# duanyiqun/DiffusionDepth

Measured on NVIDIA H100. Metric: depth maps/sec @ KITTI 352x1216, Swin-L, 20 DDIM steps, higher is better.
Workload: dtype f32 (fp32-grade products on wgmma: 3-pass fp16 split, fp32 accumulate)

## Files before the change

### diffusiondepth_b200/csrc/engine.cu

```cuda
#include <cuda.h>
#include <cuda_runtime.h>
#include <math.h>
#include <stdio.h>
#include <stdlib.h>
#include <string.h>

#include <algorithm>
#include <map>
#include <string>
#include <vector>

#include "../../include/dd_engine.h"
#include "kernels.cuh"
#include "convgen.cuh"
#include "conv_halo.cuh"
#include "pred_fold.cuh"
#include "swin.cuh"
#include "mpvit.cuh"
#include "backward.cuh"
#include "codec_train.cuh"
#include "producer_train.cuh"

namespace {

// ... 289 lines not shown
  float* UP[3] = {nullptr, nullptr, nullptr};
  bool resample = false;
  float* UPR[3] = {nullptr, nullptr, nullptr};
  float* KS = nullptr;
};
struct ResBlockW {
  GenLayer c1, c2, ds;
  bool has_ds = false;
};
struct ResNetW {
  bool enabled = false, ready = false;
  int H = 0, W = 0;
  int depths[4] = {0, 0, 0, 0}, C[4] = {64, 128, 256, 512}, Hs[4] = {0, 0, 0, 0}, Ws[4] = {0, 0, 0, 0};
  std::vector<ResBlockW> blocks[4];
  Planes IN, T, Yp[2];
  float* Y32[2] = {nullptr, nullptr};
  float* D32 = nullptr;
};

struct DwLayer {
  int C = 0, K = 3;
  float* w = nullptr;
  float* bias = nullptr;
  int bn = -1;
  float *raw_w = nullptr, *raw_bias = nullptr;
};
struct MpBlockW {
  float *ln1_g = nullptr, *ln1_b = nullptr, *ln2_g = nullptr, *ln2_b = nullptr;
  GenLayer qkv, proj, fc1, fc2;
};
struct MpEncoderW {
  DwLayer cpe;
  float* crpe_w = nullptr;
  float* crpe_b = nullptr;
  std::vector<MpBlockW> layers;
};
struct MpStageW {
  DwLayer pe_dw[4], inv_dw;
  GenLayer pe_pw[4], inv1, inv2, agg;
  MpEncoderW enc[4];
};
constexpr int kMpHeads = 8;
constexpr int kMpChunksMax = 256;
struct FactorAttBufs {
  float *part_m = nullptr, *part_s = nullptr, *colinv = nullptr, *part_ktv = nullptr, *ktv = nullptr;
};
struct MPViTW {
  bool enabled = false, ready = false;
  int H = 0, W = 0, heads = kMpHeads, mlp_ratio = 4;
  int dims[4] = {0, 0, 0, 0}, out_dims[4] = {0, 0, 0, 0}, layers[4] = {0, 0, 0, 0}, paths[4] = {0, 0, 0, 0};
  int Hs[4] = {0, 0, 0, 0}, Ws[4] = {0, 0, 0, 0};
  GenLayer stem0, stem1;
  MpStageW stage[4];
  Planes IN, S1, D, EP0, AP, HP, CAT;
  float* XS = nullptr;
  float* E[4] = {nullptr, nullptr, nullptr, nullptr};
  float* R1 = nullptr;
  float* QKV = nullptr;
  FactorAttBufs fab;
};

struct DropPathState {
  int mask[4] = {0, 0, 0, 0}, blocks = 0;
  bool on = false;
  float* scales = nullptr;
};

}

struct dd_engine {
  dd_config cfg;
  int sm_count = 0;
  bool weights_ready = false;
  bool packed = false;
  std::map<std::string, Raw> raw;
  ConvLayer L[12];
  struct Fold {
    __half* w = nullptr;
    float* bias = nullptr;
    float wscale = 1.f;
    float* src[2] = {nullptr, nullptr};
    double* k5 = nullptr;
    float* k5_abs = nullptr;
  } fold;
  float* w_flip[6] = {};
  float* amax = nullptr;
  PackStage* stage = nullptr;
  cudaEvent_t pack_done = nullptr;
  float* gn_gamma[4] = {nullptr, nullptr, nullptr, nullptr};
  float* gn_beta[4] = {nullptr, nullptr, nullptr, nullptr};
  float* temb = nullptr;
  float* dec_wt = nullptr;
  float* dec_bt = nullptr;
  float* dec_wc = nullptr;
  float dec_bc = 0.f;
  float* dec_wu = nullptr;
  float* dec_bu = nullptr;
  float* dec_bn = nullptr;
  float *enc_w1 = nullptr, *enc_b1 = nullptr, *enc_w2 = nullptr, *enc_b2 = nullptr;
  int codec_mode = DD_CODEC_EVAL;
  struct CodecTrain {
    float *dec_gb = nullptr;
    float *dec_wt = nullptr, *dec_bt = nullptr, *dec_bn = nullptr;
    float* zero16 = nullptr;
    float *enc_w1 = nullptr, *enc_w2 = nullptr, *enc_gb = nullptr;
    float *enc_w1f = nullptr, *enc_b1f = nullptr, *enc_w2f = nullptr, *enc_b2f = nullptr;
    double *part = nullptr, *sum1 = nullptr;
    double *sums = nullptr, *part_db = nullptr;
    float* rec = nullptr;
    int nrec = 0;
  } ct;
  int producer_mode = DD_PRODUCER_EVAL;
  struct ProdBn {
    GenLayer raw;
    float *gamma = nullptr, *beta = nullptr;
    int C = 0;
    int stage = 0;
    long long n = 0;
    bool fresh = false;
    size_t rec_off = 0;
    std::string key;
  };
  struct ProdTrain {
    std::vector<ProdBn> layers;
    float* U = nullptr;
    double *part = nullptr, *sum1 = nullptr;
    float *s = nullptr, *t = nullptr, *rec = nullptr;
    size_t rec_floats = 0;
  } pt;
  struct BnSync {
    dd_allgather_fn fn = nullptr;
    void* user = nullptr;
    int world = 1;
    int cap = 0;
    double *row = nullptr, *rows = nullptr, *tot1 = nullptr, *tot2 = nullptr;
  } sync;
  std::vector<void*> owned;
  std::vector<int64_t> ts;
  std::vector<float> cx, ce;
  void* ws = nullptr;
  float *x32 = nullptr, *Y = nullptr, *cond = nullptr, *mr[4] = {}, *temb_sel = nullptr;
  double* stats[4] = {};
  __half *xs_hi = nullptr, *xs_lo = nullptr, *S_hi[2] = {}, *S_lo[2] = {};
  int* status = nullptr;
  struct Bwd {
    float *y1 = nullptr, *y2 = nullptr, *y5 = nullptr, *y6 = nullptr;
    Planes a1, f0, fa, fp, a5;
    float *g[2] = {nullptr, nullptr};
    Planes gp;
    float *gn_part = nullptr, *ab = nullptr, *col_part = nullptr, *dtemb = nullptr, *dcond = nullptr;
    float *scales = nullptr, *amax = nullptr;
    double* wg_part = nullptr;
  } bw;
  struct LoopBwd {
    float* stash = nullptr;
    float* gl = nullptr;
    float* stage = nullptr;
    double* acc = nullptr;
    double* acc_cond = nullptr;
    float *z = nullptr, *r = nullptr, *du = nullptr;
    double *part_act = nullptr, *part_wc = nullptr, *part_wt = nullptr;
  } lp;
  int stats_tiles_img[4] = {0, 0, 0, 0};
  Producers prod;
  Backbone bb;
  ResNetW rn;
// ... 398 lines not shown
  return launched(e, "gn_finalize");
}

template <int C, int COND>
void launch_apply(const dd::ApplyArgs& a, int B, int up_qpb, cudaStream_t st) {
  if (COND == 2 && C == 256) {
    if (up_qpb == 4) {
      dim3 grid((a.W / 2 + 1 + 3) / 4, a.H / 2 + 1, B);
      dd::gn_apply_up_split_kernel<4, 4><<<grid, 256, 0, st>>>(a);
    } else {
      dim3 grid(a.W / 2 + 1, a.H / 2 + 1, B);
      dd::gn_apply_up_split_kernel<4, 1><<<grid, 64, 0, st>>>(a);
    }
  } else {
    constexpr int PPB = 256 / (C / 8);
    dim3 grid((a.H * a.W + PPB - 1) / PPB, B);
    dd::gn_apply_split_kernel<C, COND><<<grid, 256, 0, st>>>(a);
  }
}

template <int C, int COND>
int run_apply(dd_engine* e, int which, const float* temb, int temb_bstride, __half* out_hi, __half* out_lo,
              cudaStream_t st, const float* y = nullptr) {
  const Geom g = geom_of(e->cfg);
  dd::ApplyArgs a;
  a.y = y != nullptr ? y : e->Y;
  a.mean_rstd = e->mr[which];
  a.gamma = e->gn_gamma[which];
  a.beta = e->gn_beta[which];
  a.cond = e->cond;
  a.temb = temb;
  a.temb_bstride = temb_bstride;
  a.H = g.h;
  a.W = g.w;
  a.ch = e->cfg.cond_h;
  a.cw = e->cfg.cond_w;
  a.ry = g.h > 1 ? static_cast<float>(a.ch - 1) / static_cast<float>(g.h - 1) : 0.f;
  a.rx = g.w > 1 ? static_cast<float>(a.cw - 1) / static_cast<float>(g.w - 1) : 0.f;
  a.out_hi = out_hi;
  a.out_lo = out_lo;
  a.scale = kActScale;
  a.status = e->status;
  launch_apply<C, COND>(a, g.B, 4, st);
  return launched(e, "gn_apply");
}

bool fold_active(const dd_engine* e) {
  return e->cfg.variant == DD_VARIANT_SWIN && !(e->cfg.flags & (DD_FLAG_SIMT_CONV | DD_FLAG_CHAIN_PRED));
}
int ring_blocks_per_img(const Geom& g) {
  return std::min(dd::ring_segments(g.h, g.w), g.tiles_max / g.B);
}

int run_fold(dd_engine* e, cudaStream_t st) {
  const Geom g = geom_of(e->cfg);
  int rc;
  CUtensorMap m_hi, m_lo;
  if ((rc = make_patch_map(&m_hi, e->S_hi[0], g.B, g.h, g.w))) return rc;
  if ((rc = make_patch_map(&m_lo, e->S_lo[0], g.B, g.h, g.w))) return rc;
  dd::FoldArgs a;
  a.B = g.B;
  a.H = g.h;
  a.W = g.w;
  a.tiles_x = (g.w + dd::F5_TW - 1) / dd::F5_TW;
  a.tiles_y = (g.h + dd::F5_TH - 1) / dd::F5_TH;
  a.num_tiles = a.tiles_x * a.tiles_y * g.B;
  a.w = e->fold.w;
  a.bias = e->fold.bias;
  a.acc_scale = 1.f / (kActScale * e->fold.wscale);
  a.y32 = e->Y;
  a.stats_partial = e->stats[2];
  e->stats_tiles_img[2] = a.tiles_x * a.tiles_y;
  const int grid = std::min(a.num_tiles, e->sm_count);
  dd::conv5x5_fold_kernel<<<grid, dd::F5::THREADS, dd::F5::SMEM_BYTES, st>>>(m_hi, m_lo, a);
  if ((rc = launched(e, "conv5x5_fold"))) return rc;
  dd::RingArgs r;
  r.H = g.h;
  r.W = g.w;
  r.nseg = dd::ring_segments(g.h, g.w);
  r.blocks_per_img = ring_blocks_per_img(g);
  r.a_hi = e->S_hi[0];
  r.a_lo = e->S_lo[0];
  r.a_inv_scale = 1.f / kActScale;
  r.wb = e->L[3].w_simt;
  r.bb = e->L[3].bias;
  r.wp = e->L[4].w_simt;
  r.y32 = e->Y;
  r.ring_partial = e->stats[3];
  dd::ring_fix_kernel<<<dim3(r.blocks_per_img, g.B), dd::RING_THREADS, dd::RING_SMEM, st>>>(r);
  return launched(e, "ring_fix");
}

int run_tail(dd_engine* e, float cx, float ce, float* eps_out, cudaStream_t st);

void launch_final(const dd::FinalArgs& f, int B, cudaStream_t st) {
  dim3 grid((f.P * 4 + 255) / 256, B);
  dd::gn_relu_ddim_kernel<<<grid, 256, 0, st>>>(f);
}

int run_step(dd_engine* e, const float* temb, int temb_bstride, float cx, float ce, float* eps_out, cudaStream_t st) {
  const Geom g = geom_of(e->cfg);
  int rc;
  if ((rc = run_conv(e, 0, e->xs_hi, e->xs_lo, kXScale, dd::EPI_F32_STATS, e->Y, e->stats[0], nullptr, nullptr, st))) return rc;
  if ((rc = run_finalize(e, 0, 64, st))) return rc;
  if ((rc = run_apply<64, 0>(e, 0, nullptr, 0, e->S_hi[0], e->S_lo[0], st))) return rc;
  if ((rc = run_conv(e, 1, e->S_hi[0], e->S_lo[0], kActScale, dd::EPI_F32_STATS, e->Y, e->stats[1], nullptr, nullptr, st)))
    return rc;
  if ((rc = run_finalize(e, 1, 256, st))) return rc;
  const __half *p_hi, *p_lo;
  if (e->cfg.variant == DD_VARIANT_SWIN) {
    if ((rc = run_apply<256, 2>(e, 1, temb, temb_bstride, e->S_hi[1], e->S_lo[1], st))) return rc;
    if ((rc = run_conv(e, 2, e->S_hi[1], e->S_lo[1], kActScale, dd::EPI_SPLIT, nullptr, nullptr, e->S_hi[0], e->S_lo[0], st)))
      return rc;
    if (fold_active(e)) {
      if ((rc = run_fold(e, st))) return rc;
      if ((rc = run_finalize(e, 2, 64, st, e->stats[3], ring_blocks_per_img(g)))) return rc;
      return run_tail(e, cx, ce, eps_out, st);
    }
    if ((rc = run_conv(e, 3, e->S_hi[0], e->S_lo[0], kActScale, dd::EPI_SPLIT, nullptr, nullptr, e->S_hi[1], e->S_lo[1], st)))
      return rc;
    p_hi = e->S_hi[1];
    p_lo = e->S_lo[1];
  } else {
    if ((rc = run_apply<256, 1>(e, 1, temb, temb_bstride, e->S_hi[1], e->S_lo[1], st))) return rc;
    p_hi = e->S_hi[1];
    p_lo = e->S_lo[1];
  }
  if ((rc = run_conv(e, 4, p_hi, p_lo, kActScale, dd::EPI_F32_STATS, e->Y, e->stats[2], nullptr, nullptr, st))) return rc;
  if ((rc = run_finalize(e, 2, 64, st))) return rc;
  return run_tail(e, cx, ce, eps_out, st);
}

int run_tail(dd_engine* e, float cx, float ce, float* eps_out, cudaStream_t st) {
  const Geom g = geom_of(e->cfg);
  int rc;
  if ((rc = run_apply<64, 0>(e, 2, nullptr, 0, e->S_hi[0], e->S_lo[0], st))) return rc;
  if ((rc = run_conv(e, 5, e->S_hi[0], e->S_lo[0], kActScale, dd::EPI_F32_STATS, e->Y, e->stats[3], nullptr, nullptr, st))) return rc;
  if ((rc = run_finalize(e, 3, 16, st))) return rc;
  dd::FinalArgs f;
  f.y = e->Y;
  f.mean_rstd = e->mr[3];
  f.gamma = e->gn_gamma[3];
  f.beta = e->gn_beta[3];
  f.x = e->x32;
  f.x_hi = e->xs_hi;
  f.x_lo = e->xs_lo;
  f.eps_out = eps_out;
  f.cx = cx;
  f.ce = ce;
  f.scale = kXScale;
  f.P = g.P;
  f.status = e->status;
  launch_final(f, g.B, st);
  return launched(e, "gn_relu_ddim");
}

int transpose_in(const float* nchw, float* nhwc, int B, int C, int P, cudaStream_t st) {
  dim3 grid((P + 31) / 32, (C + 31) / 32, B), block(32, 8);
  dd::nchw_to_nhwc_kernel<<<grid, block, 0, st>>>(nchw, nhwc, C, P);
  return check_launch("nchw_to_nhwc");
}
int transpose_out(const float* nhwc, float* nchw, int B, int C, int P, cudaStream_t st) {
  dim3 grid((P + 31) / 32, (C + 31) / 32, B), block(32, 8);
  dd::nhwc_to_nchw_kernel<<<grid, block, 0, st>>>(nhwc, nchw, C, P);
  return check_launch("nhwc_to_nchw");
}
int split_planes(dd_engine* e, const float* x, __half* hi, __half* lo, size_t n, float scale, cudaStream_t st) {
  dd::split_planes_kernel<<<grid_of(n / 4), 256, 0, st>>>(x, hi, lo, n / 4, scale, e->status);
  return check_launch("split_planes");
// ... 145 lines not shown
int bn_fold(const float* const* bn, int ch, std::vector<float>& scale, std::vector<float>& shift, cudaStream_t st) {
  std::vector<float> v[4];
  for (int i = 0; i < 4; ++i) {
    v[i].resize(ch);
    CUDA_TRY(cudaMemcpyAsync(v[i].data(), bn[i], ch * 4, cudaMemcpyDeviceToHost, st));
  }
  CUDA_TRY(cudaStreamSynchronize(st));
  scale.resize(ch);
  shift.resize(ch);
  const float* host[4] = {v[0].data(), v[1].data(), v[2].data(), v[3].data()};
  bn_fold_host(host, ch, scale.data(), shift.data());
  return DD_OK;
}
int find_bn(dd_engine* e, const std::string& prefix, const float** bn) {
  const char* parts[4] = {".weight", ".bias", ".running_mean", ".running_var"};
  for (int i = 0; i < 4; ++i) {
    const Raw* r = find(e, prefix + parts[i]);
    if (!r) return fail(DD_ERR_INVALID, "missing weights: " + prefix + parts[i]);
    bn[i] = r->ptr;
  }
  return DD_OK;
}
int copy_param(dd_engine* e, const std::string& key, size_t n, float** out, cudaStream_t st) {
  const Raw* r = find(e, key);
  if (!r) return fail(DD_ERR_INVALID, "missing weights: " + key);
  size_t have = 1;
  for (int64_t d : r->shape) have *= static_cast<size_t>(d);
  if (have != n) return fail(DD_ERR_INVALID, "weight shape mismatch: " + key);
  int rc;
  if ((rc = dev_alloc(e, reinterpret_cast<void**>(out), n * 4))) return rc;
  CUDA_TRY(cudaMemcpyAsync(*out, r->ptr, n * 4, cudaMemcpyDeviceToDevice, st));
  return DD_OK;
}

const char* const kGnKey[4] = {"model.noise_embedding.1", "model.noise_embedding.4", "model.pred.1", "model.pred.4"};
constexpr int kGnCh[4] = {64, 256, 64, 16};
const std::string kDecPrefix = "depth_transform.conv_inv_transform.";
const std::string kEncPrefix = "depth_transform.conv_transform.";
struct CodecKey {
  const char* leaf;
  size_t host_off;
  std::vector<int64_t> shape;
};
#define DD_STAGE_OFF(m) (offsetof(PackStage, m) / sizeof(float))
const CodecKey kDecKeys[8] = {{"0.weight", DD_STAGE_OFF(dec_wt), {16, 16, 4, 4}}, {"0.bias", DD_STAGE_OFF(dec_bt), {16}},
                              {"1.weight", DD_STAGE_OFF(dec_g), {16}},            {"1.bias", DD_STAGE_OFF(dec_be), {16}},
                              {"1.running_mean", DD_STAGE_OFF(dec_mu), {16}},     {"1.running_var", DD_STAGE_OFF(dec_var), {16}},
                              {"3.0.weight", DD_STAGE_OFF(dec_wc), {1, 16, 3, 3}}, {"3.0.bias", DD_STAGE_OFF(dec_bc), {1}}};
const CodecKey kEncKeys[10] = {
    {"0.0.weight", DD_STAGE_OFF(enc_w1), {16, 1, 3, 3}},        {"0.1.weight", DD_STAGE_OFF(enc_bn1[0]), {16}},
    {"0.1.bias", DD_STAGE_OFF(enc_bn1[1]), {16}},               {"0.1.running_mean", DD_STAGE_OFF(enc_bn1[2]), {16}},
    {"0.1.running_var", DD_STAGE_OFF(enc_bn1[3]), {16}},        {"1.0.weight", DD_STAGE_OFF(enc_w2), {16, 16, 3, 3}},
    {"1.1.weight", DD_STAGE_OFF(enc_bn2[0]), {16}},             {"1.1.bias", DD_STAGE_OFF(enc_bn2[1]), {16}},
    {"1.1.running_mean", DD_STAGE_OFF(enc_bn2[2]), {16}},       {"1.1.running_var", DD_STAGE_OFF(enc_bn2[3]), {16}}};
#undef DD_STAGE_OFF
size_t numel(const std::vector<int64_t>& s) {
  size_t n = 1;
  for (int64_t d : s) n *= static_cast<size_t>(d);
  return n;
}

int alloc_pack(dd_engine* h, bool encoder, cudaStream_t st) {
  const bool swin = h->cfg.variant == DD_VARIANT_SWIN;
  int rc;
  if ((rc = dev_array(h, &h->amax, 16))) return rc;
  for (int i = 0; i < 6; ++i) {
    if (!swin && (i == 2 || i == 3)) continue;
    const int co = kConvCout[i], ci = kConvCin[i];
    if ((rc = alloc_layer(h, h->L[i], co, ci))) return rc;
    if (has_backward(h->cfg)) {
      if ((rc = dev_array(h, &h->w_flip[i], static_cast<size_t>(co) * ci * 9))) return rc;
      if ((rc = alloc_layer(h, h->L[6 + i], ci, co))) return rc;
      CUDA_TRY(cudaMemsetAsync(h->L[6 + i].bias, 0, ci * 4, st));
    }
  }
  if (fold_active(h)) {
    const size_t n5 = 64 * 256 * 25;
    if ((rc = dev_array(h, &h->fold.w, dd::F5::W_ELEMS))) return rc;
    if ((rc = dev_array(h, &h->fold.bias, 64))) return rc;
    if ((rc = dev_array(h, &h->fold.src[0], 256 * 256 * 9))) return rc;
    if ((rc = dev_array(h, &h->fold.src[1], 64 * 256 * 9))) return rc;
    if ((rc = dev_array(h, &h->fold.k5, n5))) return rc;
    if ((rc = dev_array(h, &h->fold.k5_abs, n5))) return rc;
  }
  for (int i = 0; i < 4; ++i) {
    if ((rc = dev_array(h, &h->gn_gamma[i], kGnCh[i]))) return rc;
    if ((rc = dev_array(h, &h->gn_beta[i], kGnCh[i]))) return rc;
  }
  if ((rc = dev_array(h, &h->temb, DD_TIME_ROWS * 256))) return rc;
  if ((rc = dev_array(h, &h->dec_wt, 4 * 4 * 16 * 16))) return rc;
  if ((rc = dev_array(h, &h->dec_bt, 16))) return rc;
  if ((rc = dev_array(h, &h->dec_wc, 9 * 16))) return rc;
  if ((rc = dev_array(h, &h->dec_wu, 4 * 4 * 16 * 16))) return rc;
  if ((rc = dev_array(h, &h->dec_bu, 16))) return rc;
  if ((rc = dev_array(h, &h->dec_bn, 3 * 16))) return rc;
  dd_engine::CodecTrain& ct = h->ct;
  if ((rc = dev_array(h, &ct.dec_gb, 2 * 16))) return rc;
  if ((rc = dev_array(h, &ct.dec_wt, 4 * 4 * 16 * 16))) return rc;
  if ((rc = dev_array(h, &ct.dec_bt, 16))) return rc;
  if ((rc = dev_array(h, &ct.dec_bn, 3 * 16))) return rc;
  if ((rc = dev_array(h, &ct.zero16, 16))) return rc;
  CUDA_TRY(cudaMemsetAsync(ct.zero16, 0, 16 * 4, st));
  const Geom g = geom_of(h->cfg);
  if ((rc = dev_array(h, &ct.part, static_cast<size_t>(codec_stats_blocks(static_cast<long long>(g.B) * g.P * 4)) *
                                         dd::BNS_COLS)))
    return rc;
  if ((rc = dev_array(h, &ct.sum1, 16))) return rc;
  if ((rc = dev_array(h, &ct.sums, 32))) return rc;
  if ((rc = dev_array(h, &ct.part_db, static_cast<size_t>(dec_act_blocks(g)) * 16))) return rc;
  if ((rc = dev_array(h, &ct.rec, static_cast<size_t>(std::max(h->cfg.num_inference_steps, 2)) * 32))) return rc;
  ct.nrec = 0;
  h->enc_w1 = nullptr;
  if (encoder) {
    if ((rc = dev_array(h, &h->enc_w1, 144))) return rc;
    if ((rc = dev_array(h, &h->enc_b1, 16))) return rc;
    if ((rc = dev_array(h, &h->enc_w2, 2304))) return rc;
    if ((rc = dev_array(h, &h->enc_b2, 16))) return rc;
    if ((rc = dev_array(h, &ct.enc_w1, 144))) return rc;
    if ((rc = dev_array(h, &ct.enc_w2, 2304))) return rc;
    if ((rc = dev_array(h, &ct.enc_gb, 4 * 16))) return rc;
    if ((rc = dev_array(h, &ct.enc_w1f, 144))) return rc;
    if ((rc = dev_array(h, &ct.enc_b1f, 16))) return rc;
    if ((rc = dev_array(h, &ct.enc_w2f, 2304))) return rc;
    if ((rc = dev_array(h, &ct.enc_b2f, 16))) return rc;
  }
  return DD_OK;
}

int check_update(dd_engine* h) {
  const bool swin = h->cfg.variant == DD_VARIANT_SWIN;
  std::map<std::string, std::vector<int64_t>> want;
  for (int i = 0; i < 6; ++i) {
    if (!swin && (i == 2 || i == 3)) continue;
    want[std::string(kConvKey[i]) + ".weight"] = {kConvCout[i], kConvCin[i], 3, 3};
    want[std::string(kConvKey[i]) + ".bias"] = {kConvCout[i]};
  }
  for (int i = 0; i < 4; ++i) want[std::string(kGnKey[i]) + ".weight"] = want[std::string(kGnKey[i]) + ".bias"] = {kGnCh[i]};
  want["model.time_embedding.weight"] = {DD_TIME_ROWS, 256};
  for (const CodecKey& k : kDecKeys) want[kDecPrefix + k.leaf] = k.shape;
  if (h->enc_w1)
    for (const CodecKey& k : kEncKeys) want[kEncPrefix + k.leaf] = k.shape;
  for (const auto& kv : h->raw) {
    const std::string& name = kv.first;
    for (const char* p : {"hahineck.", "conv_lateral.", "conv_up.", "backbone."})
      if (name.compare(0, strlen(p), p) == 0)
        return fail(DD_ERR_UNSUPPORTED, name + ": the neck, FPN and backbone are re-packed by dd_finalize_weights only");
    auto it = want.find(name);
    if (it == want.end()) return fail(DD_ERR_INVALID, name + " is not part of this engine's pack");
    if (kv.second.shape != it->second) return fail(DD_ERR_INVALID, name + ": shape differs from the packed tensor");
  }
  return DD_OK;
}

bool loop_reads_wscale(const dd_engine* e, int layer) { return !(fold_active(e) && (layer == 3 || layer == 4)); }

int fill_pack(dd_engine* h, cudaStream_t st) {
  const bool swin = h->cfg.variant == DD_VARIANT_SWIN;
  PackStage* sg = h->stage;
  float* sg_f = reinterpret_cast<float*>(sg);
  auto W = [&](const std::string& k) -> const float* {
    const Raw* r = find(h, k);
    return r ? r->ptr : nullptr;
  };
  int rc;
  CUDA_TRY(cudaStreamWaitEvent(st, h->pack_done, 0));
  CUDA_TRY(cudaMemsetAsync(h->amax, 0, 16 * 4, st));
  const float* w[6] = {};
  bool fold = false;
  for (int i = 0; i < 6; ++i) {
    if (!swin && (i == 2 || i == 3)) continue;
    const int co = kConvCout[i], ci = kConvCin[i];
    const int n = co * ci * 9;
    w[i] = W(std::string(kConvKey[i]) + ".weight");
    const float* b = W(std::string(kConvKey[i]) + ".bias");
    if (b) CUDA_TRY(cudaMemcpyAsync(h->L[i].bias, b, co * 4, cudaMemcpyDeviceToDevice, st));
    if (w[i]) {
      dd::absmax_kernel<<<absmax_grid(n), 256, 0, st>>>(w[i], n, h->amax + i);
      if ((rc = check_launch("absmax"))) return rc;
      if (has_backward(h->cfg)) {
        dd::flip_transpose_weight_kernel<<<64, 256, 0, st>>>(w[i], h->w_flip[i], co, ci);
        if ((rc = check_launch("flip_transpose_weight"))) return rc;
        dd::absmax_kernel<<<absmax_grid(n), 256, 0, st>>>(h->w_flip[i], n, h->amax + 6 + i);
        if ((rc = check_launch("absmax"))) return rc;
      }
    }
    if (fold_active(h) && (i == 3 || i == 4)) {
      if (w[i]) CUDA_TRY(cudaMemcpyAsync(h->fold.src[i - 3], w[i], static_cast<size_t>(n) * 4, cudaMemcpyDeviceToDevice, st));
      fold |= w[i] || b;
    }
  }
  if (fold) {
    dd::compose_fold_kernel<<<256, 256, 0, st>>>(h->fold.src[1], h->L[4].bias, h->fold.src[0], h->L[3].bias, h->fold.k5,
                                                 h->fold.k5_abs, h->fold.bias);
    if ((rc = check_launch("compose_fold"))) return rc;
    dd::absmax_kernel<<<absmax_grid(64 * 256 * 25), 256, 0, st>>>(h->fold.k5_abs, 64 * 256 * 25, h->amax + 12);
    if ((rc = check_launch("absmax"))) return rc;
  }
  for (int i = 0; i < 4; ++i) {
    if (const float* g = W(std::string(kGnKey[i]) + ".weight"))
      CUDA_TRY(cudaMemcpyAsync(h->gn_gamma[i], g, kGnCh[i] * 4, cudaMemcpyDeviceToDevice, st));
    if (const float* b = W(std::string(kGnKey[i]) + ".bias"))
      CUDA_TRY(cudaMemcpyAsync(h->gn_beta[i], b, kGnCh[i] * 4, cudaMemcpyDeviceToDevice, st));
  }
  if (const float* t = W("model.time_embedding.weight"))
    CUDA_TRY(cudaMemcpyAsync(h->temb, t, DD_TIME_ROWS * 256 * 4, cudaMemcpyDeviceToDevice, st));
  bool dec = false, enc = false;
  for (const CodecKey& k : kDecKeys)
    if (const float* p = W(kDecPrefix + k.leaf)) {
      CUDA_TRY(cudaMemcpyAsync(sg_f + k.host_off, p, numel(k.shape) * 4, cudaMemcpyDeviceToHost, st));
      dec = true;
    }
  if (h->enc_w1)
    for (const CodecKey& k : kEncKeys)
      if (const float* p = W(kEncPrefix + k.leaf)) {
        CUDA_TRY(cudaMemcpyAsync(sg_f + k.host_off, p, numel(k.shape) * 4, cudaMemcpyDeviceToHost, st));
        enc = true;
      }
  CUDA_TRY(cudaMemcpyAsync(sg->amax, h->amax, 16 * 4, cudaMemcpyDeviceToHost, st));
  CUDA_TRY(cudaStreamSynchronize(st));

  bool loop_stale = false, steps_stale = false;
  for (int i = 0; i < 6; ++i) {
    if (!w[i]) continue;
    const int co = kConvCout[i], ci = kConvCin[i];
    ConvLayer& L = h->L[i];
    const float s = dd::grad_scale_of(sg->amax[i]);
    loop_stale |= s != L.wscale && loop_reads_wscale(h, i);
    L.wscale = s;
    dd::pack_conv_weight_kernel<<<128, 256, 0, st>>>(w[i], L.w_hi, L.w_lo, L.w_simt, co, ci, L.wscale);
    if ((rc = check_launch("pack_conv_weight"))) return rc;
    if (has_backward(h->cfg)) {
      ConvLayer& D = h->L[6 + i];
      D.wscale = dd::grad_scale_of(sg->amax[6 + i]);
      dd::pack_conv_weight_kernel<<<128, 256, 0, st>>>(h->w_flip[i], D.w_hi, D.w_lo, D.w_simt, ci, co, D.wscale);
      if ((rc = check_launch("pack_conv_weight"))) return rc;
    }
  }
  if (fold) {
    const float s = dd::grad_scale_of(sg->amax[12]);
    loop_stale |= s != h->fold.wscale;
    h->fold.wscale = s;
    dd::pack_fold_kernel<<<256, 256, 0, st>>>(h->fold.k5, h->fold.w, static_cast<double>(h->fold.wscale));
    if ((rc = check_launch("pack_fold"))) return rc;
  }
  if (dec) {
    for (int co = 0; co < 16; ++co) {
      const double sc = static_cast<double>(sg->dec_g[co]) / sqrt(static_cast<double>(sg->dec_var[co]) + 1e-5);
      sg->bt_f[co] = static_cast<float>((static_cast<double>(sg->dec_bt[co]) - sg->dec_mu[co]) * sc + sg->dec_be[co]);
      for (int ci = 0; ci < 16; ++ci)
        for (int ky = 0; ky < 4; ++ky)
          for (int kx = 0; kx < 4; ++kx)
            sg->wt_f[((ky * 4 + kx) * 16 + ci) * 16 + co] =
                static_cast<float>(static_cast<double>(sg->dec_wt[((ci * 16 + co) * 4 + ky) * 4 + kx]) * sc);
    }
    for (int ci = 0; ci < 16; ++ci)
      for (int tap = 0; tap < 9; ++tap) sg->wc_f[tap * 16 + ci] = sg->dec_wc[ci * 9 + tap];
    CUDA_TRY(cudaMemcpyAsync(h->dec_wt, sg->wt_f, sizeof(sg->wt_f), cudaMemcpyHostToDevice, st));
    CUDA_TRY(cudaMemcpyAsync(h->dec_bt, sg->bt_f, sizeof(sg->bt_f), cudaMemcpyHostToDevice, st));
    CUDA_TRY(cudaMemcpyAsync(h->dec_wc, sg->wc_f, sizeof(sg->wc_f), cudaMemcpyHostToDevice, st));
    steps_stale |= sg->dec_bc[0] != h->dec_bc;
    h->dec_bc = sg->dec_bc[0];
    for (int co = 0; co < 16; ++co) {
      const double rstd = 1.0 / sqrt(static_cast<double>(sg->dec_var[co]) + 1e-5);
      sg->bn[co] = static_cast<float>(static_cast<double>(sg->dec_g[co]) * rstd);
      sg->bn[16 + co] = sg->dec_mu[co];
      sg->bn[32 + co] = static_cast<float>(rstd);
      for (int ci = 0; ci < 16; ++ci)
        for (int k = 0; k < 16; ++k) sg->wu[(k * 16 + ci) * 16 + co] = sg->dec_wt[(ci * 16 + co) * 16 + k];
    }
    CUDA_TRY(cudaMemcpyAsync(h->dec_wu, sg->wu, sizeof(sg->wu), cudaMemcpyHostToDevice, st));
    CUDA_TRY(cudaMemcpyAsync(h->dec_bu, sg->dec_bt, sizeof(sg->dec_bt), cudaMemcpyHostToDevice, st));
    CUDA_TRY(cudaMemcpyAsync(h->dec_bn, sg->bn, sizeof(sg->bn), cudaMemcpyHostToDevice, st));
    CUDA_TRY(cudaMemcpyAsync(h->ct.dec_gb, sg->dec_g, 16 * 4, cudaMemcpyHostToDevice, st));
    CUDA_TRY(cudaMemcpyAsync(h->ct.dec_gb + 16, sg->dec_be, 16 * 4, cudaMemcpyHostToDevice, st));
  }
  if (enc) {
    float s1[16], s2[16];
// ... 2459 lines not shown
```

### diffusiondepth_b200/csrc/pred_fold.cuh

```cuda
#pragma once
#include "conv_common.cuh"

namespace dd {

constexpr int F5_TH = 16;
constexpr int F5_TW = 16;

struct F5 {
  static constexpr int CIN = 256, COUT = 64, BK = 16, KC = CIN / BK;
  static constexpr int PH = F5_TH + 4, PW = F5_TW + 4;
  static constexpr int XP = PH * 16;
  static constexpr int CGP = PW * XP;
  static constexpr int PLANE = 2 * CGP;
  static constexpr int P_SLOT = 2 * PLANE;
  static constexpr int P_SLOTS = 3;
  static constexpr int W_PLANE = COUT * BK * 2;
  static constexpr int W_TAP = 2 * W_PLANE;
  static constexpr int W_SLOT = 5 * W_TAP;
  static constexpr int W_SLOTS = 6;
  static constexpr int CHP = 32;
  static constexpr int LD = COUT + 4;
  static constexpr int STAGE_BYTES = 2 * CHP * LD * 4;
  static constexpr int CTRL_BYTES = 1024;
  static constexpr int SMEM_BYTES = P_SLOTS * P_SLOT + W_SLOTS * W_SLOT + CTRL_BYTES + STAGE_BYTES + 1024;
// ... 132 lines not shown
          if (dy == 4) prev_p = sp;
          if (++sw == F5::W_SLOTS) {
            sw = 0;
            pw ^= 1;
          }
        }
        if (++sp == F5::P_SLOTS) {
          sp = 0;
          pp ^= 1;
        }
      };
      for (int kc = 0; kc < F5::KC; kc += 2) {
        chunk(acc0, kc);
        chunk(acc1, kc + 1);
      }
      wgmma_wait<0>();
      wgmma_fence_regs(acc0);
      wgmma_fence_regs(acc1);
      retire_prev();

      const int tx = tile % p.tiles_x, ty = (tile / p.tiles_x) % p.tiles_y, img = tile / (p.tiles_x * p.tiles_y);
      const int x0 = tx * F5_TW, yw = ty * F5_TH + wg * 8;
      const int co0 = 16 * q + (lane >> 2);
      const float bias0 = __ldg(p.bias + co0), bias1 = __ldg(p.bias + co0 + 8);
      float tk = 0.f, tsum = 0.f, tsq = 0.f;
      int tn = 0;
#pragma unroll
      for (int cj = 0; cj < F5_TW / 4; ++cj) {
        named_bar_sync(2 + wg, 128);
#pragma unroll
        for (int ii = 0; ii < 4; ++ii) {
          const int i = 4 * cj + ii;
          const int x = x0 + i;
#pragma unroll
          for (int e = 0; e < 4; ++e) {
            const int yl = 2 * (lane & 3) + (e & 1);
            const int y = yw + yl;
            const float v = fmaf(acc0[4 * i + e] + acc1[4 * i + e], p.acc_scale, (e >> 1) ? bias1 : bias0);
            if (x > 0 && x < p.W - 1 && y > 0 && y < p.H - 1) {
              if (tn++ == 0) tk = v;
              const float d = v - tk;
              tsum += d;
              tsq = fmaf(d, d, tsq);
            }
            S[(ii * 8 + yl) * F5::LD + co0 + 8 * (e >> 1)] = v;
          }
        }
        named_bar_sync(2 + wg, 128);
#pragma unroll
        for (int k = 0; k < 4; ++k) {
          const int n = 8 * q + 2 * k + (lane >> 4);
          const int x = x0 + 4 * cj + (n >> 3), y = yw + (n & 7);
          if (x < p.W && y < p.H) {
            const float4 v = *reinterpret_cast<const float4*>(S + n * F5::LD + 4 * (lane & 15));
            *reinterpret_cast<float4*>(p.y32 + ((static_cast<size_t>(img) * p.H + y) * p.W + x) * F5::COUT +
                                       4 * (lane & 15)) = v;
          }
        }
      }
      const double n = tn, kk = tk, ds = tsum;
      double s = fma(n, kk, ds), s2 = fma(n * kk, kk, fma(2.0 * kk, ds, static_cast<double>(tsq)));
#pragma unroll
      for (int o = 16; o > 0; o >>= 1) {
        s += __shfl_xor_sync(0xffffffffu, s, o);
        s2 += __shfl_xor_sync(0xffffffffu, s2, o);
      }
      if (lane == 0) {
        red[((par * 2 + wg) * 4 + q) * 2 + 0] = s;
        red[((par * 2 + wg) * 4 + q) * 2 + 1] = s2;
      }
      named_bar_sync(1, 256);
      const int e = threadIdx.x - 128;
      if (e < 8) {
        const int g = e >> 1, which = e & 1;
        p.stats_partial[(static_cast<size_t>(tile) * 4 + g) * 2 + which] =
            red[((par * 2 + 0) * 4 + g) * 2 + which] + red[((par * 2 + 1) * 4 + g) * 2 + which];
      }
      par ^= 1;
    }
  }
}

constexpr int RING_S = 16;
constexpr int RING_BOX = RING_S + 2;
constexpr int RING_ABOX = RING_S + 4;
constexpr int RING_JG = 4;
constexpr int RING_JB = (RING_BOX + RING_JG - 1) / RING_JG;
constexpr int RING_THREADS = 256 * RING_JG;
constexpr int RING_SMEM = (5 * RING_ABOX + 3 * RING_BOX + 4) * 256 * 4 + RING_S * 64 * 4;

struct RingSide {
  int y0, x0, vert, len;
};
__host__ __device__ inline int ring_sides(int H, int W, RingSide* s) {
  int n = 0;
  if (H <= 2) {
    for (int y = 0; y < H; ++y) s[n++] = {y, 0, 0, W};
  } else if (W <= 2) {
    for (int x = 0; x < W; ++x) s[n++] = {0, x, 1, H};
  } else {
    s[n++] = {0, 0, 0, W};
    s[n++] = {H - 1, 0, 0, W};
    s[n++] = {1, 0, 1, H - 2};
    s[n++] = {1, W - 1, 1, H - 2};
  }
  return n;
}
__host__ __device__ inline int ring_segments(int H, int W) {
  RingSide s[4];
  const int n = ring_sides(H, W, s);
  int k = 0;
  for (int i = 0; i < n; ++i) k += (s[i].len + RING_S - 1) / RING_S;
  return k;
}

struct RingArgs {
  int H, W;
  int nseg, blocks_per_img;
  const __half* a_hi;
  const __half* a_lo;
  float a_inv_scale;
  const float* wb;
  const float* bb;
  const float* wp;
  float* y32;
  double* ring_partial;
};

__device__ __forceinline__ bool inside_img(int y, int x, int H, int W) { return y >= 0 && y < H && x >= 0 && x < W; }

__global__ void __launch_bounds__(RING_THREADS) ring_fix_kernel(const RingArgs p) {
  extern __shared__ float4 ring_smem4[];
  float* abox = reinterpret_cast<float*>(ring_smem4);
  float* bbox = abox + 5 * RING_ABOX * 256;
  double* red = reinterpret_cast<double*>(bbox + 3 * RING_BOX * 256);
  float* ycor = bbox + (3 * RING_BOX + 4) * 256;
  const int img = blockIdx.y, t = threadIdx.x;
  const int H = p.H, W = p.W;
  RingSide sd[4];
  ring_sides(H, W, sd);
  const int s_begin = static_cast<int>(static_cast<long long>(p.nseg) * blockIdx.x / p.blocks_per_img);
  const int s_end = static_cast<int>(static_cast<long long>(p.nseg) * (blockIdx.x + 1) / p.blocks_per_img);
  double ts = 0.0, tq = 0.0;
  for (int sg = s_begin; sg < s_end; ++sg) {
    int k = sg, si = 0;
    while (k >= (sd[si].len + RING_S - 1) / RING_S) {
      k -= (sd[si].len + RING_S - 1) / RING_S;
      ++si;
    }
    const int n = min(RING_S, sd[si].len - k * RING_S);
    const int ly = sd[si].vert, lx = 1 - ly;
    const int ay = lx, ax = ly;
    const int oy = sd[si].y0 + k * RING_S * ly, ox = sd[si].x0 + k * RING_S * lx;
    __syncthreads();
    for (int i = t; i < 5 * RING_ABOX * 32; i += RING_THREADS) {
      const int c8 = i & 31, pos = i >> 5;
      const int r = pos / RING_ABOX - 2, c = pos % RING_ABOX - 2;
      const int y = oy + r * ay + c * ly, x = ox + r * ax + c * lx;
      float v[8] = {0.f, 0.f, 0.f, 0.f, 0.f, 0.f, 0.f, 0.f};
      if (c <= n + 1 && inside_img(y, x, H, W)) {
        const size_t o = ((static_cast<size_t>(img) * H + y) * W + x) * 256 + c8 * 8;
        const uint4 hv = __ldg(reinterpret_cast<const uint4*>(p.a_hi + o));
        const uint4 lv = __ldg(reinterpret_cast<const uint4*>(p.a_lo + o));
        const __half* hh = reinterpret_cast<const __half*>(&hv);
        const __half* ll = reinterpret_cast<const __half*>(&lv);
#pragma unroll
        for (int j = 0; j < 8; ++j) v[j] = (__half2float(hh[j]) + __half2float(ll[j])) * p.a_inv_scale;
      }
      float4* d = reinterpret_cast<float4*>(abox + pos * 256 + c8 * 8);
      d[0] = make_float4(v[0], v[1], v[2], v[3]);
      d[1] = make_float4(v[4], v[5], v[6], v[7]);
    }
    __syncthreads();
    const int cm = t & 255, j0 = (t >> 8) * RING_JB;
    for (int r = -1; r <= 1; ++r) {
      uint32_t omask = 0;
      for (int j = j0; j < min(n + 2, j0 + RING_JB); ++j)
        if (!inside_img(oy + r * ay + (j - 1) * ly, ox + r * ax + (j - 1) * lx, H, W)) omask |= 1u << (j - j0);
      if (omask == 0) continue;
      float acc[RING_JB];
#pragma unroll
      for (int j = 0; j < RING_JB; ++j) acc[j] = 0.f;
      for (int tp = 0; tp < 9; ++tp) {
        const int rr = tp / 3 - 1, cc = tp % 3 - 1;
        uint32_t vmask = 0;
        for (int j = 0; j < RING_JB; ++j) {
          const int jb = j0 + j;
          if (((omask >> j) & 1u) && inside_img(oy + (r + rr) * ay + (jb - 1 + cc) * ly, ox + (r + rr) * ax + (jb - 1 + cc) * lx, H, W))
            vmask |= 1u << j;
        }
        if (vmask == 0) continue;
        const int dy = rr * ay + cc * ly, dx = rr * ax + cc * lx;
        const float* wt = p.wb + static_cast<size_t>((dy + 1) * 3 + (dx + 1)) * 65536 + cm;
        const float* arow = abox + ((r + rr + 2) * RING_ABOX + j0 + cc + 1) * 256;
#pragma unroll 4
        for (int ci = 0; ci < 256; ci += 4) {
          const float w0 = __ldg(wt + (ci + 0) * 256), w1 = __ldg(wt + (ci + 1) * 256);
          const float w2 = __ldg(wt + (ci + 2) * 256), w3 = __ldg(wt + (ci + 3) * 256);
#pragma unroll
          for (int j = 0; j < RING_JB; ++j)
            if ((vmask >> j) & 1u) {
              const float4 av = *reinterpret_cast<const float4*>(arow + j * 256 + ci);
              acc[j] = fmaf(w3, av.w, fmaf(w2, av.z, fmaf(w1, av.y, fmaf(w0, av.x, acc[j]))));
            }
        }
      }
      const float bias = __ldg(p.bb + cm);
#pragma unroll
      for (int j = 0; j < RING_JB; ++j)
        if ((omask >> j) & 1u) bbox[((r + 1) * RING_BOX + j0 + j) * 256 + cm] = acc[j] + bias;
    }
    __syncthreads();
    const int co = t & 63;
    for (int j = t >> 6; j < n; j += RING_THREADS / 64) {
      const int y = oy + j * ly, x = ox + j * lx;
      float corr = 0.f;
      for (int tp = 0; tp < 9; ++tp) {
        const int rr = tp / 3 - 1, cc = tp % 3 - 1;
        const int dy = rr * ay + cc * ly, dx = rr * ax + cc * lx;
        if (inside_img(y + dy, x + dx, H, W)) continue;
        const float* bq = bbox + ((rr + 1) * RING_BOX + j + cc + 1) * 256;
        const float* wt = p.wp + static_cast<size_t>((dy + 1) * 3 + (dx + 1)) * 256 * 64 + co;
        for (int c = 0; c < 256; c += 4) {
          const float4 b4 = *reinterpret_cast<const float4*>(bq + c);
          corr = fmaf(__ldg(wt + (c + 0) * 64), b4.x, corr);
          corr = fmaf(__ldg(wt + (c + 1) * 64), b4.y, corr);
          corr = fmaf(__ldg(wt + (c + 2) * 64), b4.z, corr);
          corr = fmaf(__ldg(wt + (c + 3) * 64), b4.w, corr);
        }
      }
      float* yp = p.y32 + ((static_cast<size_t>(img) * H + y) * W + x) * 64 + co;
      const float v = *yp - corr;
      *yp = v;
      ycor[j * 64 + co] = v;
    }
    __syncthreads();
    if (t < 256)
      for (int j = t >> 6; j < n; j += 4) {
        const double v = ycor[j * 64 + co];
        ts += v;
        tq = fma(v, v, tq);
      }
  }
  if (t < 256) {
    red[t] = ts;
    red[256 + t] = tq;
  }
  __syncthreads();
  if (t < 8) {
    const int g = t >> 1, which = t & 1;
    double s = 0.0;
    for (int pg = 0; pg < 4; ++pg)
      for (int c = 0; c < 16; ++c) s += red[which * 256 + pg * 64 + g * 16 + c];
    p.ring_partial[((static_cast<size_t>(img) * p.blocks_per_img + blockIdx.x) * 4 + g) * 2 + which] = s;
  }
}

__global__ void compose_fold_kernel(const float* __restrict__ wp, const float* __restrict__ bp,
                                    const float* __restrict__ wb, const float* __restrict__ bb,
                                    double* __restrict__ k5, float* __restrict__ k5_abs, float* __restrict__ b5) {
  const int n = 64 * 256 * 25;
  for (int i = blockIdx.x * blockDim.x + threadIdx.x; i < n; i += gridDim.x * blockDim.x) {
    const int t5 = i % 25, ci = (i / 25) % 256, co = i / (25 * 256);
    const int Dy = t5 / 5 - 2, Dx = t5 % 5 - 2;
    double s = 0.0;
    for (int cm = 0; cm < 256; ++cm)
      for (int ky = 0; ky < 3; ++ky) {
        const int ey = Dy - (ky - 1);
        if (ey < -1 || ey > 1) continue;
        for (int kx = 0; kx < 3; ++kx) {
          const int ex = Dx - (kx - 1);
          if (ex < -1 || ex > 1) continue;
          s += static_cast<double>(wp[((co * 256 + cm) * 3 + ky) * 3 + kx]) *
               static_cast<double>(wb[((cm * 256 + ci) * 3 + ey + 1) * 3 + ex + 1]);
        }
      }
    k5[i] = s;
    k5_abs[i] = static_cast<float>(fabs(s));
    if (ci == 0 && t5 == 0) {
      double b = bp[co];
      for (int cm = 0; cm < 256; ++cm)
        for (int k = 0; k < 9; ++k) b += static_cast<double>(wp[(co * 256 + cm) * 9 + k]) * static_cast<double>(bb[cm]);
      b5[co] = static_cast<float>(b);
    }
  }
}
__global__ void pack_fold_kernel(const double* __restrict__ k5, __half* __restrict__ out, double scale) {
  const int n = 64 * 256 * 25;
  for (int i = blockIdx.x * blockDim.x + threadIdx.x; i < n; i += gridDim.x * blockDim.x) {
    const int t5 = i % 25, ci = (i / 25) % 256, co = i / (25 * 256);
    const double v = k5[i] * scale;
    const __half hi = __float2half_rn(static_cast<float>(v));
    const __half lo = __float2half_rn(static_cast<float>(v - static_cast<double>(__half2float(hi))));
    const int kc = ci / 16, kg = (ci / 8) & 1, k8 = ci & 7;
    const size_t base = static_cast<size_t>((kc * 25 + t5) * 2) * 2;
    const size_t cm = static_cast<size_t>((co >> 3) * 64 + (co & 7) * 8 + k8);
    out[(base + 0 + kg) * 512 + cm] = hi;
    out[(base + 2 + kg) * 512 + cm] = lo;
  }
}

}
```

Baseline: 27.07.

## Precompose border-correction weights for ring fix instead of recomputing intermediate conv

The ring-fix kernel corrects the folded 5x5 conv at image borders. Previously it recomputed the intermediate 3x3 conv activations around each border segment and then applied the second 3x3 conv's missing taps. It now uses precomposed edge, corner and bias-constant weight tables, built once at weight-load time by a new compose_edge kernel, and applies them as 1D 5-tap convolutions along the border line. Corners get separate inclusion-exclusion terms. This removes a large amount of per-step 256x256 FMA work and shared memory. The cost is a new composed-weight table and a more intricate correction that relies on the algebra being exactly right.

```diff
diff --git a/diffusiondepth_b200/csrc/engine.cu b/diffusiondepth_b200/csrc/engine.cu
--- a/diffusiondepth_b200/csrc/engine.cu
+++ b/diffusiondepth_b200/csrc/engine.cu
@@ -395,6 +395,7 @@
     float* src[2] = {nullptr, nullptr};
     double* k5 = nullptr;
     float* k5_abs = nullptr;
+    float* edge = nullptr;
   } fold;
   float* w_flip[6] = {};
   float* amax = nullptr;
@@ -959,9 +960,7 @@
   r.a_hi = e->S_hi[0];
   r.a_lo = e->S_lo[0];
   r.a_inv_scale = 1.f / kActScale;
-  r.wb = e->L[3].w_simt;
-  r.bb = e->L[3].bias;
-  r.wp = e->L[4].w_simt;
+  r.edge = e->fold.edge;
   r.y32 = e->Y;
   r.ring_partial = e->stats[3];
   dd::ring_fix_kernel<<<dim3(r.blocks_per_img, g.B), dd::RING_THREADS, dd::RING_SMEM, st>>>(r);
@@ -1273,6 +1272,7 @@
     if ((rc = dev_array(h, &h->fold.src[1], 64 * 256 * 9))) return rc;
     if ((rc = dev_array(h, &h->fold.k5, n5))) return rc;
     if ((rc = dev_array(h, &h->fold.k5_abs, n5))) return rc;
+    if ((rc = dev_array(h, &h->fold.edge, dd::EDGE_ELEMS))) return rc;
   }
   for (int i = 0; i < 4; ++i) {
     if ((rc = dev_array(h, &h->gn_gamma[i], kGnCh[i]))) return rc;
@@ -1384,6 +1384,8 @@
     dd::compose_fold_kernel<<<256, 256, 0, st>>>(h->fold.src[1], h->L[4].bias, h->fold.src[0], h->L[3].bias, h->fold.k5,
                                                  h->fold.k5_abs, h->fold.bias);
     if ((rc = check_launch("compose_fold"))) return rc;
+    dd::compose_edge_kernel<<<256, 256, 0, st>>>(h->fold.src[1], h->fold.src[0], h->L[3].bias, h->fold.edge);
+    if ((rc = check_launch("compose_edge"))) return rc;
     dd::absmax_kernel<<<absmax_grid(64 * 256 * 25), 256, 0, st>>>(h->fold.k5_abs, 64 * 256 * 25, h->amax + 12);
     if ((rc = check_launch("absmax"))) return rc;
   }
diff --git a/diffusiondepth_b200/csrc/pred_fold.cuh b/diffusiondepth_b200/csrc/pred_fold.cuh
--- a/diffusiondepth_b200/csrc/pred_fold.cuh
+++ b/diffusiondepth_b200/csrc/pred_fold.cuh
@@ -238,12 +238,13 @@
 }
 
 constexpr int RING_S = 16;
-constexpr int RING_BOX = RING_S + 2;
-constexpr int RING_ABOX = RING_S + 4;
-constexpr int RING_JG = 4;
-constexpr int RING_JB = (RING_BOX + RING_JG - 1) / RING_JG;
-constexpr int RING_THREADS = 256 * RING_JG;
-constexpr int RING_SMEM = (5 * RING_ABOX + 3 * RING_BOX + 4) * 256 * 4 + RING_S * 64 * 4;
+constexpr int RING_LINE = RING_S + 4;
+constexpr int RING_THREADS = 256;
+constexpr int RING_KQ = 5 * 256 / 4;
+constexpr int RING_SMEM = RING_LINE * 256 * 4 + 4 * RING_S * 64 * 4 + 4 * 64 * 4 + 2 * 256 * 8;
+constexpr int EDGE_E = 5 * 256 * 64;
+constexpr int EDGE_C = 256 * 64;
+constexpr int EDGE_ELEMS = 4 * EDGE_E + 4 * EDGE_C + 8 * 64;
 
 struct RingSide {
   int y0, x0, vert, len;
@@ -276,27 +277,34 @@
   const __half* a_hi;
   const __half* a_lo;
   float a_inv_scale;
-  const float* wb;
-  const float* bb;
-  const float* wp;
+  const float* edge;
   float* y32;
   double* ring_partial;
 };
 
 __device__ __forceinline__ bool inside_img(int y, int x, int H, int W) { return y >= 0 && y < H && x >= 0 && x < W; }
+__device__ __forceinline__ bool on_side(int s, int y, int x, int H, int W) {
+  return s == 0 ? y == 0 : s == 1 ? y == H - 1 : s == 2 ? x == 0 : x == W - 1;
+}
 
 __global__ void __launch_bounds__(RING_THREADS) ring_fix_kernel(const RingArgs p) {
   extern __shared__ float4 ring_smem4[];
-  float* abox = reinterpret_cast<float*>(ring_smem4);
-  float* bbox = abox + 5 * RING_ABOX * 256;
-  double* red = reinterpret_cast<double*>(bbox + 3 * RING_BOX * 256);
-  float* ycor = bbox + (3 * RING_BOX + 4) * 256;
+  float* line = reinterpret_cast<float*>(ring_smem4);
+  float* corr = line + RING_LINE * 256;
+  float* part = corr + RING_S * 64;
+  float* xred = part + 3 * RING_S * 64;
+  double* red = reinterpret_cast<double*>(xred + 4 * 64);
   const int img = blockIdx.y, t = threadIdx.x;
   const int H = p.H, W = p.W;
+  const float* cst = p.edge + 4 * EDGE_E + 4 * EDGE_C;
   RingSide sd[4];
   ring_sides(H, W, sd);
   const int s_begin = static_cast<int>(static_cast<long long>(p.nseg) * blockIdx.x / p.blocks_per_img);
   const int s_end = static_cast<int>(static_cast<long long>(p.nseg) * (blockIdx.x + 1) / p.blocks_per_img);
+  auto a_at = [&](int y, int x, int ci) {
+    const size_t o = ((static_cast<size_t>(img) * H + y) * W + x) * 256 + ci;
+    return (__half2float(p.a_hi[o]) + __half2float(p.a_lo[o])) * p.a_inv_scale;
+  };
   double ts = 0.0, tq = 0.0;
   for (int sg = s_begin; sg < s_end; ++sg) {
     int k = sg, si = 0;
@@ -306,13 +314,12 @@
     }
     const int n = min(RING_S, sd[si].len - k * RING_S);
     const int ly = sd[si].vert, lx = 1 - ly;
-    const int ay = lx, ax = ly;
     const int oy = sd[si].y0 + k * RING_S * ly, ox = sd[si].x0 + k * RING_S * lx;
+    const int s0 = 2 * ly;
     __syncthreads();
-    for (int i = t; i < 5 * RING_ABOX * 32; i += RING_THREADS) {
+    for (int i = t; i < RING_LINE * 32; i += RING_THREADS) {
       const int c8 = i & 31, pos = i >> 5;
-      const int r = pos / RING_ABOX - 2, c = pos % RING_ABOX - 2;
-      const int y = oy + r * ay + c * ly, x = ox + r * ax + c * lx;
+      const int c = pos - 2, y = oy + c * ly, x = ox + c * lx;
       float v[8] = {0.f, 0.f, 0.f, 0.f, 0.f, 0.f, 0.f, 0.f};
       if (c <= n + 1 && inside_img(y, x, H, W)) {
         const size_t o = ((static_cast<size_t>(img) * H + y) * W + x) * 256 + c8 * 8;
@@ -323,85 +330,113 @@
 #pragma unroll
         for (int j = 0; j < 8; ++j) v[j] = (__half2float(hh[j]) + __half2float(ll[j])) * p.a_inv_scale;
       }
-      float4* d = reinterpret_cast<float4*>(abox + pos * 256 + c8 * 8);
+      float4* d = reinterpret_cast<float4*>(line + pos * 256 + c8 * 8);
       d[0] = make_float4(v[0], v[1], v[2], v[3]);
       d[1] = make_float4(v[4], v[5], v[6], v[7]);
     }
     __syncthreads();
-    const int cm = t & 255, j0 = (t >> 8) * RING_JB;
-    for (int r = -1; r <= 1; ++r) {
-      uint32_t omask = 0;
-      for (int j = j0; j < min(n + 2, j0 + RING_JB); ++j)
-        if (!inside_img(oy + r * ay + (j - 1) * ly, ox + r * ax + (j - 1) * lx, H, W)) omask |= 1u << (j - j0);
-      if (omask == 0) continue;
-      float acc[RING_JB];
-#pragma unroll
-      for (int j = 0; j < RING_JB; ++j) acc[j] = 0.f;
-      for (int tp = 0; tp < 9; ++tp) {
-        const int rr = tp / 3 - 1, cc = tp % 3 - 1;
-        uint32_t vmask = 0;
-        for (int j = 0; j < RING_JB; ++j) {
-          const int jb = j0 + j;
-          if (((omask >> j) & 1u) && inside_img(oy + (r + rr) * ay + (jb - 1 + cc) * ly, ox + (r + rr) * ax + (jb - 1 + cc) * lx, H, W))
-            vmask |= 1u << j;
-        }
-        if (vmask == 0) continue;
-        const int dy = rr * ay + cc * ly, dx = rr * ax + cc * lx;
-        const float* wt = p.wb + static_cast<size_t>((dy + 1) * 3 + (dx + 1)) * 65536 + cm;
-        const float* arow = abox + ((r + rr + 2) * RING_ABOX + j0 + cc + 1) * 256;
-#pragma unroll 4
-        for (int ci = 0; ci < 256; ci += 4) {
-          const float w0 = __ldg(wt + (ci + 0) * 256), w1 = __ldg(wt + (ci + 1) * 256);
-          const float w2 = __ldg(wt + (ci + 2) * 256), w3 = __ldg(wt + (ci + 3) * 256);
-#pragma unroll
-          for (int j = 0; j < RING_JB; ++j)
-            if ((vmask >> j) & 1u) {
-              const float4 av = *reinterpret_cast<const float4*>(arow + j * 256 + ci);
-              acc[j] = fmaf(w3, av.w, fmaf(w2, av.z, fmaf(w1, av.y, fmaf(w0, av.x, acc[j]))));
-            }
-        }
-      }
-      const float bias = __ldg(p.bb + cm);
-#pragma unroll
-      for (int j = 0; j < RING_JB; ++j)
-        if ((omask >> j) & 1u) bbox[((r + 1) * RING_BOX + j0 + j) * 256 + cm] = acc[j] + bias;
+    {
+      const int kq = t >> 6, cg = t & 15, pg = (t >> 4) & 3;
+      float acc[4][4];
+#pragma unroll
+      for (int i = 0; i < 4; ++i)
+#pragma unroll
+        for (int c = 0; c < 4; ++c) acc[i][c] = 0.f;
+      for (int s = s0; s < s0 + 2; ++s) {
+        if (!on_side(s, oy, ox, H, W)) continue;
+        const float* E = p.edge + s * EDGE_E + 4 * cg;
+#pragma unroll 2
+        for (int kk = kq * RING_KQ; kk < (kq + 1) * RING_KQ; kk += 4) {
+          const int tap = kk >> 8, ci = kk & 255;
+          float4 w[4];
+#pragma unroll
+          for (int r = 0; r < 4; ++r) w[r] = __ldg(reinterpret_cast<const float4*>(E + (kk + r) * 64));
+#pragma unroll
+          for (int i = 0; i < 4; ++i) {
+            const float4 av = *reinterpret_cast<const float4*>(line + (4 * pg + i + tap) * 256 + ci);
+            acc[i][0] = fmaf(av.w, w[3].x, fmaf(av.z, w[2].x, fmaf(av.y, w[1].x, fmaf(av.x, w[0].x, acc[i][0]))));
+            acc[i][1] = fmaf(av.w, w[3].y, fmaf(av.z, w[2].y, fmaf(av.y, w[1].y, fmaf(av.x, w[0].y, acc[i][1]))));
+            acc[i][2] = fmaf(av.w, w[3].z, fmaf(av.z, w[2].z, fmaf(av.y, w[1].z, fmaf(av.x, w[0].z, acc[i][2]))));
+            acc[i][3] = fmaf(av.w, w[3].w, fmaf(av.z, w[2].w, fmaf(av.y, w[1].w, fmaf(av.x, w[0].w, acc[i][3]))));
+          }
+        }
+      }
+      if (kq > 0)
+#pragma unroll
+        for (int i = 0; i < 4; ++i)
+          *reinterpret_cast<float4*>(part + ((kq - 1) * RING_S + 4 * pg + i) * 64 + 4 * cg) =
+              make_float4(acc[i][0], acc[i][1], acc[i][2], acc[i][3]);
+      __syncthreads();
+      if (kq == 0) {
+        float c0[4] = {0.f, 0.f, 0.f, 0.f};
+        for (int s = s0; s < s0 + 2; ++s)
+          if (on_side(s, oy, ox, H, W))
+#pragma unroll
+            for (int c = 0; c < 4; ++c) c0[c] += cst[s * 64 + 4 * cg + c];
+#pragma unroll
+        for (int i = 0; i < 4; ++i) {
+          float v[4] = {acc[i][0], acc[i][1], acc[i][2], acc[i][3]};
+#pragma unroll
+          for (int q = 0; q < 3; ++q) {
+            const float4 h = *reinterpret_cast<const float4*>(part + (q * RING_S + 4 * pg + i) * 64 + 4 * cg);
+            v[0] += h.x;
+            v[1] += h.y;
+            v[2] += h.z;
+            v[3] += h.w;
+          }
+          *reinterpret_cast<float4*>(corr + (4 * pg + i) * 64 + 4 * cg) =
+              make_float4(v[0] + c0[0], v[1] + c0[1], v[2] + c0[2], v[3] + c0[3]);
+        }
+      }
     }
     __syncthreads();
-    const int co = t & 63;
-    for (int j = t >> 6; j < n; j += RING_THREADS / 64) {
+    for (int e = 0; e < 2; ++e) {
+      const int j = e == 0 ? (ly ? -oy : -ox) : (ly ? H - 1 - oy : W - 1 - ox);
+      if (j < 0 || j >= n || (e == 1 && j == (ly ? -oy : -ox))) continue;
       const int y = oy + j * ly, x = ox + j * lx;
-      float corr = 0.f;
-      for (int tp = 0; tp < 9; ++tp) {
-        const int rr = tp / 3 - 1, cc = tp % 3 - 1;
-        const int dy = rr * ay + cc * ly, dx = rr * ax + cc * lx;
-        if (inside_img(y + dy, x + dx, H, W)) continue;
-        const float* bq = bbox + ((rr + 1) * RING_BOX + j + cc + 1) * 256;
-        const float* wt = p.wp + static_cast<size_t>((dy + 1) * 3 + (dx + 1)) * 256 * 64 + co;
-        for (int c = 0; c < 256; c += 4) {
-          const float4 b4 = *reinterpret_cast<const float4*>(bq + c);
-          corr = fmaf(__ldg(wt + (c + 0) * 64), b4.x, corr);
-          corr = fmaf(__ldg(wt + (c + 1) * 64), b4.y, corr);
-          corr = fmaf(__ldg(wt + (c + 2) * 64), b4.z, corr);
-          corr = fmaf(__ldg(wt + (c + 3) * 64), b4.w, corr);
-        }
-      }
-      float* yp = p.y32 + ((static_cast<size_t>(img) * H + y) * W + x) * 64 + co;
-      const float v = *yp - corr;
+      const int co = t & 63, c0 = (t >> 6) * 64;
+      float v = 0.f, cv = 0.f;
+      for (int s = 2 - s0; s < 4 - s0; ++s) {
+        if (!on_side(s, y, x, H, W)) continue;
+        if (t < 64) cv += cst[s * 64 + co];
+        const int ay = s >= 2, ax = s < 2;
+        for (int tap = 0; tap < 5; ++tap) {
+          const int yy = y + (tap - 2) * ay, xx = x + (tap - 2) * ax;
+          if (!inside_img(yy, xx, H, W)) continue;
+          const float* E = p.edge + s * EDGE_E + tap * 256 * 64 + co;
+          for (int ci = c0; ci < c0 + 64; ++ci) v = fmaf(a_at(yy, xx, ci), __ldg(E + ci * 64), v);
+        }
+      }
+      for (int cn = 0; cn < 4; ++cn) {
+        if (y != ((cn >> 1) ? H - 1 : 0) || x != ((cn & 1) ? W - 1 : 0)) continue;
+        if (t < 64) cv -= cst[(4 + cn) * 64 + co];
+        const float* C = p.edge + 4 * EDGE_E + cn * EDGE_C + co;
+        for (int ci = c0; ci < c0 + 64; ++ci) v = fmaf(-a_at(y, x, ci), __ldg(C + ci * 64), v);
+      }
+      xred[t] = v;
+      __syncthreads();
+      if (t < 64) corr[j * 64 + co] += xred[co] + xred[64 + co] + xred[128 + co] + xred[192 + co] + cv;
+      __syncthreads();
+    }
+    for (int i = t; i < n * 64; i += RING_THREADS) {
+      const int j = i >> 6, co = i & 63;
+      float* yp = p.y32 + ((static_cast<size_t>(img) * H + oy + j * ly) * W + ox + j * lx) * 64 + co;
+      const float v = *yp - corr[i];
       *yp = v;
-      ycor[j * 64 + co] = v;
+      part[i] = v;
     }
     __syncthreads();
-    if (t < 256)
+    {
+      const int co = t & 63;
       for (int j = t >> 6; j < n; j += 4) {
-        const double v = ycor[j * 64 + co];
+        const double v = part[j * 64 + co];
         ts += v;
         tq = fma(v, v, tq);
       }
-  }
-  if (t < 256) {
-    red[t] = ts;
-    red[256 + t] = tq;
-  }
+    }
+  }
+  red[t] = ts;
+  red[256 + t] = tq;
   __syncthreads();
   if (t < 8) {
     const int g = t >> 1, which = t & 1;
@@ -441,6 +476,41 @@
     }
   }
 }
+__global__ void compose_edge_kernel(const float* __restrict__ wp, const float* __restrict__ wb,
+                                    const float* __restrict__ bb, float* __restrict__ edge) {
+  auto P = [&](int co, int cm, int ky, int kx) { return static_cast<double>(wp[((co * 256 + cm) * 3 + ky) * 3 + kx]); };
+  auto Q = [&](int cm, int ci, int ey, int ex) { return static_cast<double>(wb[((cm * 256 + ci) * 3 + ey) * 3 + ex]); };
+  for (int i = blockIdx.x * blockDim.x + threadIdx.x; i < EDGE_ELEMS; i += gridDim.x * blockDim.x) {
+    const int co = i & 63;
+    double s = 0.0;
+    if (i < 4 * EDGE_E) {
+      const int ci = (i >> 6) & 255, tap = (i >> 14) % 5, side = i / EDGE_E;
+      const int o = (side & 1) ? 2 : 0;
+      for (int cm = 0; cm < 256; ++cm)
+        for (int k = 0; k < 3; ++k) {
+          const int e = tap - k;
+          if (e < 0 || e > 2) continue;
+          s += side < 2 ? P(co, cm, o, k) * Q(cm, ci, 2 - o, e) : P(co, cm, k, o) * Q(cm, ci, e, 2 - o);
+        }
+    } else if (i < 4 * EDGE_E + 4 * EDGE_C) {
+      const int j = i - 4 * EDGE_E, ci = (j >> 6) & 255, cn = j / EDGE_C;
+      const int ky = (cn >> 1) * 2, kx = (cn & 1) * 2;
+      for (int cm = 0; cm < 256; ++cm) s += P(co, cm, ky, kx) * Q(cm, ci, 2 - ky, 2 - kx);
+    } else {
+      const int c = (i - 4 * EDGE_E - 4 * EDGE_C) >> 6;
+      for (int cm = 0; cm < 256; ++cm) {
+        const double b = bb[cm];
+        if (c < 4) {
+          const int o = (c & 1) ? 2 : 0;
+          for (int k = 0; k < 3; ++k) s += (c < 2 ? P(co, cm, o, k) : P(co, cm, k, o)) * b;
+        } else {
+          s += P(co, cm, ((c - 4) >> 1) * 2, ((c - 4) & 1) * 2) * b;
+        }
+      }
+    }
+    edge[i] = static_cast<float>(s);
+  }
+}
 __global__ void pack_fold_kernel(const double* __restrict__ k5, __half* __restrict__ out, double scale) {
   const int n = 64 * 256 * 25;
   for (int i = blockIdx.x * blockDim.x + threadIdx.x; i < n; i += gridDim.x * blockDim.x) {
```

Result: faster. 28.19, median of 6 (+4.1%).
